# ToniChopp/ECAMP

Hardware: AMD Instinct MI355X
Metric: pretrain image-report pairs/sec (ViT-B/16, 224^2, seq=128) (higher is better)
Workload: dtype bf16

## Files before the change

ecamp_amd/csrc/attention.h:

```cpp
#pragma once
#include "common.h"

struct AttnArgs {
    const void* q; const void* k; const void* v; void* o;
    const void* dout; void* dq; void* dk; void* dv;
    float* lse; float* delta;
    const int32_t* key_mask;
    long q_sb, q_st, q_sh, k_sb, k_st, k_sh, v_sb, v_st, v_sh, o_sb, o_st, o_sh;
    long dq_sb, dq_st, dq_sh, dk_sb, dk_st, dk_sh, dv_sb, dv_st, dv_sh, do_sb, do_st, do_sh;
    int B, H, Tq, Tk;
    float scale, drop_p;
    uint64_t seed, offset;
    unsigned char* drop_bits;
};

#define NEG_BIG (-1.0e30f)

#define LDS_MAX (160 * 1024)

static inline int attn_kch(int Tk) { return Tk <= 64 ? 1 : Tk <= 128 ? 2 : Tk <= 256 ? 4 : 0; }

static inline size_t head_lds_bytes(int Tq, int Tk, int hd, bool backward, bool bits) {
    const int nkp = ((Tk + 15) / 16 + 1) / 2, nqp = ((Tq + 15) / 16 + 1) / 2;
    const size_t prow = (size_t)(backward && nqp > nkp ? nqp : nkp) * 32;
    return 2 * prow * (2 * hd) + (backward ? 3 : 1) * prow * sizeof(float) + (backward && bits ? 32 * prow : 0);
}

enum AttnFamily { ATTN_HEAD, ATTN_RESIDENT_FWD, ATTN_STREAM, ATTN_LONG, ATTN_F32 };
typedef void (*AttnKernel)(AttnArgs);
struct AttnLaunch {
    AttnFamily family;
    int n, block;
    struct Kernel { AttnKernel fn; dim3 grid; size_t lds, optin; } k[2];
};
#define ATTN_HD_SWITCH(hd, F, ...) ((hd) == 32 ? F<32>(__VA_ARGS__) : (hd) == 64 ? F<64>(__VA_ARGS__) : F<128>(__VA_ARGS__))

ECAMP_HIDDEN AttnLaunch attn16_select(int B, int H, int Tq, int Tk, int hd, bool mask_or_dropout, bool bits, bool backward);
ECAMP_HIDDEN void attn_launch(const AttnLaunch& l, const AttnArgs& a, hipStream_t st);
void attn_set_head_mode(int on);
```

ecamp_amd/csrc/attention.hip:

```cpp
#include "attention.h"


template <typename T, int HD, int PITCH>
__device__ __forceinline__ void stage_rows(float* dst, const T* base, long st, int r0, int nrows, int tid) {
    constexpr int V4 = HD / 4;
#pragma unroll
    for (int i = 0; i < (64 * V4) / 256; ++i) {
        int idx = tid + 256 * i;
        int row = idx / V4, dv = idx % V4;
        float p[4] = {0.f, 0.f, 0.f, 0.f};
        if (r0 + row < nrows) ld4<T>(base + (long)(r0 + row) * st + dv * 4, p);
        float* d = dst + row * PITCH + dv * 4;
        if (PITCH % 4 == 0) {
            *reinterpret_cast<float4*>(d) = make_float4(p[0], p[1], p[2], p[3]);
        } else {
            *reinterpret_cast<float2*>(d) = make_float2(p[0], p[1]);
            *reinterpret_cast<float2*>(d + 2) = make_float2(p[2], p[3]);
        }
    }
}

template <typename T, int HD>
__device__ __forceinline__ void load_rows_frag(float (&f)[HD / 4], const T* base, long st, int r0, int nrows, int lrow, int lk,
                                               float mul) {
// ... 450 lines not shown
                const int d = lane + 64 * t;
                if (d < HD) {
                    ak[t] = fmaf(di, qb[(long)(i0 + ii) * a.q_st + d], ak[t]);
                    av[t] = fmaf(pi, dOb[(long)(i0 + ii) * a.do_st + d], av[t]);
                }
            }
        }
    }
#pragma unroll
    for (int t = 0; t < (HD + 63) / 64; ++t) {
        const int d = lane + 64 * t;
        if (d < HD) { dk[d] = ak[t] * a.scale; dv[d] = av[t]; }
    }
}

static int attn_check(const AttnArgs& a, int hd, int dtype, bool bwd) {
    ECAMP_CHECK_ARG(hd == 32 || hd == 64 || hd == 128, "attention: head_dim %d not in {32,64,128}", hd);
    ECAMP_CHECK_ARG(a.Tk >= 1 && a.Tq >= 1, "attention: empty sequence");
    ECAMP_CHECK_ARG(dtype == ECAMP_F32 || dtype == ECAMP_BF16, "attention: bad dtype");
    ECAMP_CHECK_ARG(a.drop_p >= 0.f && a.drop_p < 1.f, "attention: bad dropout p");
    const long m = dtype == ECAMP_BF16 ? 8 : 4;
    if (dtype == ECAMP_BF16) ECAMP_CHECK_ARG(a.q_st % m == 0 && a.q_sb % m == 0 && a.q_sh % m == 0 && a.o_st % 4 == 0 && a.o_sb % 4 == 0 && a.o_sh % 4 == 0,
                                             "attention(bf16): q strides must be multiples of 8, o strides of 4 elements");
    ECAMP_CHECK_ARG(a.k_st % m == 0 && a.k_sb % m == 0 && a.k_sh % m == 0 && a.v_st % m == 0 && a.v_sb % m == 0 && a.v_sh % m == 0,
                    "attention: k/v strides must be multiples of 4 (f32) / 8 (bf16) elements");
    if (bwd) ECAMP_CHECK_ARG(a.q_st % m == 0 && a.q_sb % m == 0 && a.q_sh % m == 0 && a.do_st % m == 0 && a.do_sb % m == 0 && a.do_sh % m == 0,
                             "attention: q/dO strides must be multiples of 4 elements");
    return 0;
}

template <int HD>
static AttnLaunch select_f32(int B, int H, int Tq, int Tk, bool backward) {
    AttnLaunch l = {};
    l.family = ATTN_F32;
    l.n = backward ? 2 : 1;
    l.block = 256;
    const int kch = attn_kch(Tk);
    if (kch == 0) {
        const dim3 qrows((unsigned)(((long)B * H * Tq + 3) / 4)), krows((unsigned)(((long)B * H * Tk + 3) / 4));
        l.k[0] = {backward ? attn_long_bwd_dq_kernel<HD> : attn_long_fwd_kernel<HD>, qrows, 0, 0};
        if (backward) l.k[1] = {attn_long_bwd_dkv_kernel<HD>, krows, 0, 0};
        return l;
    }
    const dim3 qgrid(ceil_div(Tq, 64), B * H), kgrid(ceil_div(Tk, 64), B * H);
    const size_t fwd = (size_t)(64 * (HD + 16) + 4 * 16 * PP) * sizeof(float), dq = (size_t)(2 * 64 * (HD + 2) + 4 * 16 * PP) * sizeof(float),
                 dkv = (size_t)(2 * 64 * (HD + 2) + 8 * 16 * PP) * sizeof(float);
#define KCH_KERNEL(K) (kch == 1 ? K<float, HD, 1> : kch == 2 ? K<float, HD, 2> : K<float, HD, 4>)
    if (backward) {
        l.k[0] = {KCH_KERNEL(attn_bwd_dq_kernel), qgrid, dq, dq};
        l.k[1] = {attn_bwd_dkv_kernel<float, HD>, kgrid, dkv, dkv};
    } else {
        l.k[0] = {KCH_KERNEL(attn_fwd_kernel), qgrid, fwd, fwd};
    }
#undef KCH_KERNEL
    return l;
}
static AttnLaunch attn_select(int B, int H, int Tq, int Tk, int hd, int dtype, bool mask_or_dropout, bool bits, bool backward) {
    if (dtype == ECAMP_F32) return ATTN_HD_SWITCH(hd, select_f32, B, H, Tq, Tk, backward);
    return attn16_select(B, H, Tq, Tk, hd, mask_or_dropout, bits, backward);
}

static void stride3(long& sb, long& st, long& sh, const int64_t* s) {
    if (s) { sb = s[0]; st = s[1]; sh = s[2]; }
}
static AttnArgs attn_args(const void* q, const void* k, const void* v, const void* o, const void* dout, const float* lse, float* delta, void* dq,
                          void* dk, void* dv, const int32_t* key_mask, int32_t B, int32_t H, int32_t Tq, int32_t Tk, const int64_t* q_strides,
                          const int64_t* k_strides, const int64_t* v_strides, const int64_t* o_strides, const int64_t* do_strides,
                          const int64_t* dq_strides, const int64_t* dk_strides, const int64_t* dv_strides, float scale, float drop_p, uint64_t seed,
                          uint64_t offset, const void* drop_bits) {
    AttnArgs a;
    memset(&a, 0, sizeof(a));
    a.q = q; a.k = k; a.v = v; a.o = const_cast<void*>(o); a.dout = dout; a.lse = const_cast<float*>(lse); a.delta = delta;
    a.dq = dq; a.dk = dk; a.dv = dv; a.key_mask = key_mask;
    stride3(a.q_sb, a.q_st, a.q_sh, q_strides);
    stride3(a.k_sb, a.k_st, a.k_sh, k_strides);
    stride3(a.v_sb, a.v_st, a.v_sh, v_strides);
    stride3(a.o_sb, a.o_st, a.o_sh, o_strides);
    stride3(a.do_sb, a.do_st, a.do_sh, do_strides);
    stride3(a.dq_sb, a.dq_st, a.dq_sh, dq_strides);
    stride3(a.dk_sb, a.dk_st, a.dk_sh, dk_strides);
    stride3(a.dv_sb, a.dv_st, a.dv_sh, dv_strides);
    a.B = B; a.H = H; a.Tq = Tq; a.Tk = Tk; a.scale = scale; a.drop_p = drop_p; a.seed = seed; a.offset = offset;
    a.drop_bits = reinterpret_cast<unsigned char*>(const_cast<void*>(drop_bits));
    return a;
}

extern "C" int64_t ecamp_attn_mask_bytes(int32_t B, int32_t H, int32_t Tq, int32_t Tk, int32_t hd, int32_t dtype) {
    if (dtype != ECAMP_BF16 || B <= 0 || H <= 0 || Tq <= 0 || Tk <= 0 || Tk > 256) return 0;
    if (hd != 32 && hd != 64 && hd != 128) return 0;
    return ecamp_opt(OPT_ATTN_HEAD) != 0 && head_lds_bytes(Tq, Tk, hd, false, false) <= LDS_MAX ? (int64_t)B * H * Tq * 32 : 0;
}
extern "C" int ecamp_attn_fwd(const void* q, const void* k, const void* v, void* o, float* lse, const int32_t* key_mask,
                              int32_t B, int32_t H, int32_t Tq, int32_t Tk, int32_t hd, const int64_t* q_strides,
                              const int64_t* k_strides, const int64_t* v_strides, const int64_t* o_strides, float scale,
                              float drop_p, uint64_t seed, uint64_t offset, int32_t dtype, void* drop_mask, hipStream_t stream) {
    ECAMP_CHECK_ARG(q && k && v && o && lse && q_strides && k_strides && v_strides && o_strides, "attn_fwd: null pointer");
    const bool bits = dtype == ECAMP_BF16 && drop_p > 0.f && ecamp_attn_mask_bytes(B, H, Tq, Tk, hd, dtype) > 0;
    const AttnArgs a = attn_args(q, k, v, o, nullptr, lse, nullptr, nullptr, nullptr, nullptr, key_mask, B, H, Tq, Tk, q_strides, k_strides, v_strides,
                                 o_strides, nullptr, nullptr, nullptr, nullptr, scale, drop_p, seed, offset, bits ? drop_mask : nullptr);
    if (int rc = attn_check(a, hd, dtype, false)) return rc;
    const bool prof = ecamp_prof_active();
    if (prof) ecamp_prof_begin(ECAMP_PROF_ATTN, 4.0 * B * H * (double)Tq * Tk * hd, stream);
    attn_launch(attn_select(B, H, Tq, Tk, hd, dtype, key_mask != nullptr || drop_p > 0.f, a.drop_bits != nullptr, false), a, stream);
    if (prof) ecamp_prof_end(stream);
    ECAMP_LAUNCH_CHECK();
    return 0;
}

extern "C" int64_t ecamp_attn_bwd_workspace_bytes(int32_t B, int32_t H, int32_t Tq) { return (int64_t)B * H * Tq * 4; }

extern "C" int ecamp_attn_bwd(const void* q, const void* k, const void* v, const void* o, const void* dout, const float* lse,
                              float* delta_ws, void* dq, void* dk, void* dv, const int32_t* key_mask, int32_t B, int32_t H,
                              int32_t Tq, int32_t Tk, int32_t hd, const int64_t* q_strides, const int64_t* k_strides,
                              const int64_t* v_strides, const int64_t* o_strides, const int64_t* do_strides,
                              const int64_t* dq_strides, const int64_t* dk_strides, const int64_t* dv_strides, float scale,
                              float drop_p, uint64_t seed, uint64_t offset, int32_t dtype, const void* drop_mask, hipStream_t stream) {
    ECAMP_CHECK_ARG(q && k && v && o && dout && lse && delta_ws && dq && dk && dv && q_strides && k_strides && v_strides && o_strides && do_strides &&
                        dq_strides && dk_strides && dv_strides, "attn_bwd: null pointer");
    const bool bits = dtype == ECAMP_BF16 && drop_p > 0.f;
    const AttnArgs a = attn_args(q, k, v, o, dout, lse, delta_ws, dq, dk, dv, key_mask, B, H, Tq, Tk, q_strides, k_strides, v_strides, o_strides,
                                 do_strides, dq_strides, dk_strides, dv_strides, scale, drop_p, seed, offset, bits ? drop_mask : nullptr);
    if (int rc = attn_check(a, hd, dtype, true)) return rc;
    const bool prof = ecamp_prof_active();
    if (prof) ecamp_prof_begin(ECAMP_PROF_ATTN, 8.0 * B * H * (double)Tq * Tk * hd, stream);
    attn_launch(attn_select(B, H, Tq, Tk, hd, dtype, key_mask != nullptr || drop_p > 0.f, a.drop_bits != nullptr, true), a, stream);
    if (prof) ecamp_prof_end(stream);
    ECAMP_LAUNCH_CHECK();
    return 0;
}

template <typename T>
__global__ __launch_bounds__(256) void attn_probs_kernel(const T* __restrict__ q, const T* __restrict__ k, const int32_t* __restrict__ key_mask,
                                                         float* __restrict__ probs, int B, int H, int Tq, int Tk, int hd, long q_sb, long q_st,
                                                         long q_sh, long k_sb, long k_st, long k_sh, float scale) {
    const int lane = threadIdx.x & 63;
    const long row = (long)blockIdx.x * 4 + (threadIdx.x >> 6);
    if (row >= (long)B * H * Tq) return;
    const int i = (int)(row % Tq), h = (int)((row / Tq) % H), b = (int)(row / ((long)Tq * H));
    const T* qp = q + b * q_sb + i * q_st + h * q_sh;
    const T* kb = k + b * k_sb + h * k_sh;
    constexpr int MAXJ = 16;
    float s[MAXJ];
    float mx = -INFINITY;
#pragma unroll
    for (int jj = 0; jj < MAXJ; ++jj) {
        const int j = lane + 64 * jj;
        s[jj] = -INFINITY;
        if (j < Tk) {
            const T* kp = kb + (long)j * k_st;
            float acc = 0.f;
            for (int d = 0; d < hd; ++d) acc += to_f<T>(qp[d]) * to_f<T>(kp[d]);
            acc *= scale;
            if (key_mask && key_mask[(long)b * Tk + j] == 0) acc += -3.4028234663852886e38f;
            s[jj] = acc;
            mx = fmaxf(mx, acc);
        }
    }
    mx = wave_max(mx);
    float sum = 0.f;
#pragma unroll
    for (int jj = 0; jj < MAXJ; ++jj) {
        const int j = lane + 64 * jj;
        if (j < Tk) {
            s[jj] = __expf(s[jj] - mx);
            sum += s[jj];
        }
// ... 29 lines not shown
```

ecamp_amd/csrc/attention_bf16.hip:

```cpp
#include "attention.h"
#include <type_traits>

#ifdef ATTN_TS
__device__ long long attn_ts_buf[8 * 8192];
#define ATTN_STAMP(i) do { if (threadIdx.x == 0 && blockIdx.x < 8192) attn_ts_buf[blockIdx.x * 8 + (i)] = wall_clock64(); } while (0)
#else
#define ATTN_STAMP(i) do { } while (0)
#endif

typedef __attribute__((ext_vector_type(4))) short v4s16;
typedef hw_h16x8 bf16x8_t;

#define MFMA(a, b, c) ECAMP_MFMA_16x16x32(a, b, c)

#define ATTN_LOG2E 1.4426950408889634f
#define ATTN_LN2 0.6931471805599453f
__device__ __forceinline__ float attn_exp2(float x) { return __builtin_amdgcn_exp2f(x); }

template <int HD> struct TileCfg { static constexpr int PB = HD * 2 + 32; static constexpr int BYTES = 64 * PB; };

template <int HD>
__device__ __forceinline__ void stage_tile(unsigned char* lds, const bf16_t* base, long st, int r0, int nrows, int tid) {
    constexpr int CPR = HD / 8, PB = TileCfg<HD>::PB;
#pragma unroll
// ... 490 lines not shown
                    for (int r = 0; r < 4; ++r) p[r] *= dm[r];
                }
                ptile_write4(pt, li, jt * 16 + 4 * g, p);
            }
            __builtin_amdgcn_s_waitcnt(0xc07f);
            __builtin_amdgcn_wave_barrier();
#pragma unroll
            for (int kk = 0; kk < 2; ++kk) {
                bf16x8 pf = ptile_frag(pt, li, kk * 4 + g);
#pragma unroll
                for (int dt = 0; dt < HD / 16; ++dt) o[dt] = MFMA(frag_tr<HD>(VT + c * TB, dt * 16, kk * 32, lane), pf, o[dt]);
            }
            __builtin_amdgcn_s_waitcnt(0xc07f);
            __builtin_amdgcn_wave_barrier();
        }
        if (qi < a.Tq) {
#pragma unroll
            for (int dt = 0; dt < HD / 16; ++dt) store4(ob + (long)qi * a.o_st + dt * 16 + 4 * g, o[dt], 1.0f);
        }
    }
}

template <int HD> struct HeadCfg {
    static constexpr int RB = HD * 2, CPR = HD / 8;
    static constexpr unsigned long long KEYS = HD == 32 ? 0x3033030132330101ull : HD == 64 ? 0x6056142366024421ull : 0xE0CA8436CE0A3864ull;
};
template <int HD> __device__ __forceinline__ int hswz(int row) { return (int)((HeadCfg<HD>::KEYS >> (4 * (row & 15))) & 15ull); }
template <int HD> __device__ __forceinline__ unsigned haddr(int row, int chunk) {
    return (unsigned)(row * HeadCfg<HD>::RB + ((chunk ^ hswz<HD>(row)) << 4));
}
template <int HD>
__device__ __forceinline__ void head_stage(unsigned char* img, const bf16_t* base, long st, int nrows, int prow, int tid, int nthr) {
    constexpr int CPR = HeadCfg<HD>::CPR;
    const int n = prow * CPR;
    for (int i0 = tid; i0 < n; i0 += 4 * nthr) {
        uint4 v[4];
#pragma unroll
        for (int u = 0; u < 4; ++u) {
            const int idx = i0 + u * nthr, row = idx / CPR, ch = idx % CPR;
            v[u] = (idx < n && row < nrows) ? *reinterpret_cast<const uint4*>(base + (long)row * st + ch * 8) : make_uint4(0, 0, 0, 0);
        }
#pragma unroll
        for (int u = 0; u < 4; ++u) {
            const int idx = i0 + u * nthr, row = idx / CPR, ch = idx % CPR;
            if (idx < n) *reinterpret_cast<uint4*>(img + haddr<HD>(row, ch)) = v[u];
        }
    }
}
template <int HD, int U>
__device__ __forceinline__ void head_stage_pair(unsigned char* imgA, const bf16_t* baseA, long stA, unsigned char* imgB, const bf16_t* baseB, long stB,
                                                int nrows, int prow, int tid, int nthr) {
    constexpr int CPR = HeadCfg<HD>::CPR;
    const int n = prow * CPR;
    for (int i0 = tid; i0 < n; i0 += U * nthr) {
        uint4 va[U], vb[U];
#pragma unroll
        for (int u = 0; u < U; ++u) {
            const int idx = i0 + u * nthr, row = idx / CPR, ch = idx % CPR;
            const bool in = idx < n && row < nrows;
            va[u] = in ? *reinterpret_cast<const uint4*>(baseA + (long)row * stA + ch * 8) : make_uint4(0, 0, 0, 0);
            vb[u] = in ? *reinterpret_cast<const uint4*>(baseB + (long)row * stB + ch * 8) : make_uint4(0, 0, 0, 0);
        }
#pragma unroll
        for (int u = 0; u < U; ++u) {
            const int idx = i0 + u * nthr, row = idx / CPR, ch = idx % CPR;
            if (idx < n) {
                *reinterpret_cast<uint4*>(imgA + haddr<HD>(row, ch)) = va[u];
                *reinterpret_cast<uint4*>(imgB + haddr<HD>(row, ch)) = vb[u];
            }
        }
    }
}
typedef float f32x2 __attribute__((ext_vector_type(2)));
__device__ __forceinline__ f32x2 hexp2(f32x2 x) { return (f32x2){attn_exp2(x[0]), attn_exp2(x[1])}; }
__device__ __forceinline__ uint32_t hpk(f32x2 v) { return pack_bf16x2(v[0], v[1]); }
__device__ __forceinline__ bf16x8 hpack8(const float (&v)[8]) {
    const uint4 u = make_uint4(pack_bf16x2(v[0], v[1]), pack_bf16x2(v[2], v[3]), pack_bf16x2(v[4], v[5]), pack_bf16x2(v[6], v[7]));
    return __builtin_bit_cast(bf16x8, u);
}
__device__ __forceinline__ void head_key_bias(float* KB, const AttnArgs& a, int b, int prow, int tid, int nthr) {
    for (int j = tid; j < prow; j += nthr)
        KB[j] = (j < a.Tk && (a.key_mask == nullptr || a.key_mask[(long)b * a.Tk + j] != 0)) ? 0.f : NEG_BIG;
}
template <int HD> struct HeadOff {
    unsigned fr[HD / 32];
    unsigned tr[HD / 16];
    __device__ __forceinline__ HeadOff(int li, int g) {
#pragma unroll
        for (int ks = 0; ks < HD / 32; ++ks) fr[ks] = haddr<HD>(li, ks * 4 + g);
#pragma unroll
        for (int dt = 0; dt < HD / 16; ++dt) {
            const int cb = (dt * 16 + (li & 3) * 4) * 2;
            tr[dt] = haddr<HD>(4 * g + (li >> 2), cb >> 4) + (cb & 15);
        }
    }
};
template <int HD> __device__ __forceinline__ bf16x8 hfr(const unsigned char* img, const HeadOff<HD>& o, int t, int ks) {
    return *reinterpret_cast<const bf16x8*>(img + o.fr[ks] + t * (16 * HeadCfg<HD>::RB));
}
template <int HD> __device__ __forceinline__ bf16x8 htr(const unsigned char* img, const HeadOff<HD>& o, int pp, int dt) {
    const unsigned char* p = img + o.tr[dt] + pp * (32 * HeadCfg<HD>::RB);
    v4s16 lo = __builtin_amdgcn_ds_read_tr16_b64_v4i16((v4s16 __attribute__((address_space(3)))*)(p));
    v4s16 hi = __builtin_amdgcn_ds_read_tr16_b64_v4i16((v4s16 __attribute__((address_space(3)))*)(p + 16 * HeadCfg<HD>::RB));
    return (bf16x8){lo[0], lo[1], lo[2], lo[3], hi[0], hi[1], hi[2], hi[3]};
}

template <int HD, int FLAGS>
__global__ __launch_bounds__(512, 4) void attn_head_fwd_kernel(AttnArgs a) {
    extern __shared__ __attribute__((aligned(16))) unsigned char smem[];
    constexpr int RB = HeadCfg<HD>::RB;
    const int nthr = blockDim.x, nw = nthr >> 6;
    const int nkp = (((a.Tk + 15) >> 4) + 1) >> 1, prow = nkp * 32;
    const int pfull = FLAGS ? 0 : a.Tk >> 5;
    unsigned char* KI = smem;
    unsigned char* VI = smem + prow * RB;
    float* KB = reinterpret_cast<float*>(smem + 2 * prow * RB);
    const int tid = threadIdx.x, lane = tid & 63, wave = tid >> 6, li = lane & 15, g = lane >> 4;
    const int b = blockIdx.x / a.H, h = blockIdx.x % a.H;
    const long bh = blockIdx.x;
    const bf16_t* qb = reinterpret_cast<const bf16_t*>(a.q) + b * a.q_sb + h * a.q_sh;
    const bf16_t* kb = reinterpret_cast<const bf16_t*>(a.k) + b * a.k_sb + h * a.k_sh;
    const bf16_t* vb = reinterpret_cast<const bf16_t*>(a.v) + b * a.v_sb + h * a.v_sh;
    bf16_t* ob = reinterpret_cast<bf16_t*>(a.o) + b * a.o_sb + h * a.o_sh;
    bf16x8 qf[HD / 32];
    if (wave * 16 < a.Tq) load_row_frags<HD>(qf, qb, a.q_st, wave * 16, a.Tq, lane);
    head_stage_pair<HD, 4>(KI, kb, a.k_st, VI, vb, a.v_st, a.Tk, prow, tid, nthr);
    head_key_bias(KB, a, b, prow, tid, nthr);
    __syncthreads();
    const HeadOff<HD> off(li, g);
    const float sc2 = a.scale * ATTN_LOG2E;
    const float inv_keep = a.drop_p > 0.f ? 1.0f / (1.0f - a.drop_p) : 1.0f;
    for (int q0 = wave * 16; q0 < a.Tq; q0 += nw * 16) {
        auto scores = [&](int t, bool biased) {
            f32x4 acc = {0.f, 0.f, 0.f, 0.f};
#pragma unroll
            for (int ks = 0; ks < HD / 32; ++ks) acc = MFMA(hfr<HD>(KI, off, t, ks), qf[ks], acc);
            if (biased) {
                const f32x4 kb4 = *reinterpret_cast<const f32x4*>(KB + t * 16 + 4 * g);
#pragma unroll
                for (int r = 0; r < 4; ++r) acc[r] = fmaf(acc[r], sc2, kb4[r]);
            } else {
#pragma unroll
                for (int r = 0; r < 4; ++r) acc[r] *= sc2;
            }
            return acc;
        };
        float mx = NEG_BIG;
#pragma unroll 2
        for (int pp = 0; pp < pfull; ++pp) {
            const f32x4 s0 = scores(2 * pp, false), s1 = scores(2 * pp + 1, false);
            mx = fmaxf(fmaxf(fmaxf(mx, fmaxf(s0[0], s0[1])), fmaxf(s0[2], s0[3])), fmaxf(fmaxf(s1[0], s1[1]), fmaxf(s1[2], s1[3])));
        }
#pragma unroll 1
        for (int pp = pfull; pp < nkp; ++pp) {
            const f32x4 s0 = scores(2 * pp, true), s1 = scores(2 * pp + 1, true);
            mx = fmaxf(fmaxf(fmaxf(mx, fmaxf(s0[0], s0[1])), fmaxf(s0[2], s0[3])), fmaxf(fmaxf(s1[0], s1[1]), fmaxf(s1[2], s1[3])));
        }
        mx = red4_max(mx);
        const float mxs = fmaxf(mx, -1e29f);
        const int qi = q0 + li;
        float sum = 0.f;
        f32x4 o[HD / 16];
#pragma unroll
        for (int dt = 0; dt < HD / 16; ++dt) o[dt] = (f32x4){0.f, 0.f, 0.f, 0.f};
        auto pair = [&](int pp, bool biased) {
            const f32x4 s0 = scores(2 * pp, biased), s1 = scores(2 * pp + 1, biased);
            float p[8];
#pragma unroll
            for (int r = 0; r < 4; ++r) {
                p[r] = attn_exp2(s0[r] - mxs);
                p[4 + r] = attn_exp2(s1[r] - mxs);
                sum += p[r] + p[4 + r];
            }
            if (FLAGS && a.drop_p > 0.f) {
                float dm[4], dn[4];
                if ((a.Tk & 7) == 0) {
                    const bool odd = (g & 1) != 0;
                    const uint64_t e8 = ((((uint64_t)bh * a.Tq + qi) * (uint64_t)a.Tk) >> 3) + (uint64_t)(pp * 4 + (odd ? 2 : 0) + (g >> 1));
                    const uint4 P = philox4x32(a.seed, a.offset, e8);
                    const uint32_t r0 = (uint32_t)__builtin_amdgcn_ds_swizzle((int)(odd ? P.x : P.z), 0x401f);
                    const uint32_t r1 = (uint32_t)__builtin_amdgcn_ds_swizzle((int)(odd ? P.y : P.w), 0x401f);
                    const uint32_t wa0 = odd ? r0 : P.x, wa1 = odd ? r1 : P.y, wb0 = odd ? P.z : r0, wb1 = odd ? P.w : r1;
                    const uint32_t thr = dropout_thr(a.drop_p);
                    dm[0] = dropout_pick(wa0, 0, thr, inv_keep); dm[1] = dropout_pick(wa0, 1, thr, inv_keep);
                    dm[2] = dropout_pick(wa1, 0, thr, inv_keep); dm[3] = dropout_pick(wa1, 1, thr, inv_keep);
                    dn[0] = dropout_pick(wb0, 0, thr, inv_keep); dn[1] = dropout_pick(wb0, 1, thr, inv_keep);
                    dn[2] = dropout_pick(wb1, 0, thr, inv_keep); dn[3] = dropout_pick(wb1, 1, thr, inv_keep);
                } else {
                    attn_drop4(a, (uint64_t)bh * a.Tq + qi, pp * 32 + 4 * g, inv_keep, dm);
                    attn_drop4(a, (uint64_t)bh * a.Tq + qi, pp * 32 + 16 + 4 * g, inv_keep, dn);
                }
                unsigned bits = 0;
#pragma unroll
                for (int r = 0; r < 4; ++r) {
                    p[r] *= dm[r];
                    p[4 + r] *= dn[r];
                    bits |= (dm[r] != 0.f ? 1u << r : 0u) | (dn[r] != 0.f ? 16u << r : 0u);
                }
                if (a.drop_bits && qi < a.Tq) a.drop_bits[(((long)bh * a.Tq + qi) * 4 + g) * 8 + pp] = (unsigned char)bits;
            }
            const bf16x8 pf = hpack8(p);
#pragma unroll
            for (int dt = 0; dt < HD / 16; ++dt) o[dt] = MFMA(htr<HD>(VI, off, pp, dt), pf, o[dt]);
        };
#pragma unroll 2
        for (int pp = 0; pp < pfull; ++pp) pair(pp, false);
#pragma unroll 1
        for (int pp = pfull; pp < nkp; ++pp) pair(pp, true);
        sum = red4_sum(sum);
        if (qi < a.Tq) {
            if (g == 0) a.lse[bh * a.Tq + qi] = (mxs + __log2f(sum)) * ATTN_LN2;
            const float inv = sum > 0.f ? 1.0f / sum : 0.f;
#pragma unroll
            for (int dt = 0; dt < HD / 16; ++dt) store4(ob + (long)qi * a.o_st + dt * 16 + 4 * g, o[dt], inv);
        }
        if (q0 + nw * 16 < a.Tq) load_row_frags<HD>(qf, qb, a.q_st, q0 + nw * 16, a.Tq, lane);
    }
}

template <int HD, int FLAGS>
__global__ __launch_bounds__(256, (FLAGS == 0 && HD == 32) ? 5 : (FLAGS == 0 && HD == 64) ? 4 : 2) void attn_head_bwd_kernel(AttnArgs a) {
    extern __shared__ __attribute__((aligned(16))) unsigned char smem[];
    constexpr int RB = HeadCfg<HD>::RB;
    const int nthr = blockDim.x, nw = nthr >> 6;
    const int nkp = (((a.Tk + 15) >> 4) + 1) >> 1, nqp = (((a.Tq + 15) >> 4) + 1) >> 1, prow = max(nkp, nqp) * 32;
    const int pfull = FLAGS ? 0 : a.Tk >> 5;
    unsigned char* XI = smem;
    unsigned char* YI = smem + prow * RB;
    float* KB = reinterpret_cast<float*>(smem + 2 * prow * RB);
    float* LS = KB + prow;
    float* DL = LS + prow;
    unsigned char* MB = reinterpret_cast<unsigned char*>(DL + prow);
    const int tid = threadIdx.x, lane = tid & 63, wave = tid >> 6, li = lane & 15, g = lane >> 4;
    const int b = blockIdx.x / a.H, h = blockIdx.x % a.H;
    const long bh = blockIdx.x;
    const bool use_bits = FLAGS && a.drop_p > 0.f && a.drop_bits != nullptr;
    const bf16_t* qb = reinterpret_cast<const bf16_t*>(a.q) + b * a.q_sb + h * a.q_sh;
    const bf16_t* kb = reinterpret_cast<const bf16_t*>(a.k) + b * a.k_sb + h * a.k_sh;
    const bf16_t* vb = reinterpret_cast<const bf16_t*>(a.v) + b * a.v_sb + h * a.v_sh;
    const bf16_t* ob = reinterpret_cast<const bf16_t*>(a.o) + b * a.o_sb + h * a.o_sh;
    const bf16_t* gb = reinterpret_cast<const bf16_t*>(a.dout) + b * a.do_sb + h * a.do_sh;
    bf16_t* dqb = reinterpret_cast<bf16_t*>(a.dq) + b * a.dq_sb + h * a.dq_sh;
    bf16_t* dkb = reinterpret_cast<bf16_t*>(a.dk) + b * a.dk_sb + h * a.dk_sh;
    bf16_t* dvb = reinterpret_cast<bf16_t*>(a.dv) + b * a.dv_sb + h * a.dv_sh;
    const float sc2 = a.scale * ATTN_LOG2E;
    const float inv_keep = a.drop_p > 0.f ? 1.0f / (1.0f - a.drop_p) : 1.0f;
    const HeadOff<HD> off(li, g);

    ATTN_STAMP(0);
    bf16x8 qf[HD / 32], gf[HD / 32], of[HD / 32];
    float lse_c = 0.f;
    uint2 mw = make_uint2(0u, 0u);
    auto load_q = [&](int q0, bf16x8 (&q_)[HD / 32], bf16x8 (&g_)[HD / 32], bf16x8 (&o_)[HD / 32], float& l_) {
        load_row_frags<HD>(q_, qb, a.q_st, q0, a.Tq, lane);
        load_row_frags<HD>(g_, gb, a.do_st, q0, a.Tq, lane);
        load_row_frags<HD>(o_, ob, a.o_st, q0, a.Tq, lane);
        l_ = q0 + li < a.Tq ? a.lse[bh * a.Tq + q0 + li] : 0.f;
        if (use_bits && q0 + li < a.Tq) mw = *reinterpret_cast<const uint2*>(a.drop_bits + (((long)bh * a.Tq + q0 + li) * 4 + g) * 8);
    };
    if (wave * 16 < a.Tq) load_q(wave * 16, qf, gf, of, lse_c);
    head_stage_pair<HD, (HD == 128 ? 8 : 4)>(XI, kb, a.k_st, YI, vb, a.v_st, a.Tk, prow, tid, nthr);
    head_key_bias(KB, a, b, prow, tid, nthr);
    for (int i = ((a.Tq + 15) & ~15) + tid; i < prow; i += nthr) { LS[i] = 1e30f; DL[i] = 0.f; }
    __syncthreads();
    ATTN_STAMP(1);
    for (int q0 = wave * 16; q0 < a.Tq; q0 += nw * 16) {
        float dl = 0.f;
#pragma unroll
        for (int ks = 0; ks < HD / 32; ++ks)
#pragma unroll
            for (int e = 0; e < 8; ++e) dl += bf2f((bf16_t)gf[ks][e]) * bf2f((bf16_t)of[ks][e]);
        dl = red4_sum(dl);
        const int qi = q0 + li;
        const bool qok = qi < a.Tq;
        const float lse2 = qok ? lse_c * ATTN_LOG2E : 1e30f;
        if (g == 0) {
            LS[qi] = lse2;
            DL[qi] = qok ? dl : 0.f;
            if (qok && a.delta) a.delta[bh * a.Tq + qi] = dl;
        }
        f32x4 dq[HD / 16];
#pragma unroll
        for (int dt = 0; dt < HD / 16; ++dt) dq[dt] = (f32x4){0.f, 0.f, 0.f, 0.f};
        auto soft = [&](int pp, int hf, bool biased, const f32x4& s, const f32x4& dp, uint32_t& w0, uint32_t& w1) __attribute__((always_inline)) {
            const int t = 2 * pp + hf;
            f32x2 e0 = {s[0], s[1]}, e1 = {s[2], s[3]}, d0 = {dp[0], dp[1]}, d1 = {dp[2], dp[3]};
            const f32x2 sc = {sc2, sc2}, nl = {-lse2, -lse2}, dlv = {dl, dl};
            if (biased) {
                const f32x4 kb4 = *reinterpret_cast<const f32x4*>(KB + t * 16 + 4 * g);
                e0 = e0 * sc + ((f32x2){kb4[0], kb4[1]} + nl);
                e1 = e1 * sc + ((f32x2){kb4[2], kb4[3]} + nl);
            } else {
                e0 = e0 * sc + nl;
                e1 = e1 * sc + nl;
            }
            if (FLAGS && a.drop_p > 0.f) {
                float dm[4];
                if (use_bits) {
                    const unsigned nib = ((pp < 4 ? mw.x : mw.y) >> (8 * (pp & 3) + 4 * hf)) & 15u;
#pragma unroll
                    for (int r = 0; r < 4; ++r) dm[r] = (nib >> r) & 1u ? inv_keep : 0.f;
                } else {
                    attn_drop4(a, (uint64_t)bh * a.Tq + qi, t * 16 + 4 * g, inv_keep, dm);
                }
                d0 *= (f32x2){dm[0], dm[1]};
                d1 *= (f32x2){dm[2], dm[3]};
            }
            w0 = hpk(hexp2(e0) * (d0 - dlv));
            w1 = hpk(hexp2(e1) * (d1 - dlv));
        };
        auto pair = [&](int pp, bool biased) {
            uint32_t dsp[4];
            {
#pragma unroll
                for (int hf = 0; hf < 2; ++hf) {
                    const int t = 2 * pp + hf;
                    f32x4 s = {0.f, 0.f, 0.f, 0.f}, dp = {0.f, 0.f, 0.f, 0.f};
#pragma unroll
                    for (int ks = 0; ks < HD / 32; ++ks) {
                        s = MFMA(hfr<HD>(XI, off, t, ks), qf[ks], s);
                        dp = MFMA(hfr<HD>(YI, off, t, ks), gf[ks], dp);
                    }
                    soft(pp, hf, biased, s, dp, dsp[2 * hf], dsp[2 * hf + 1]);
                }
                const bf16x8 sf = __builtin_bit_cast(bf16x8, make_uint4(dsp[0], dsp[1], dsp[2], dsp[3]));
#pragma unroll
                for (int dt = 0; dt < HD / 16; ++dt) dq[dt] = MFMA(htr<HD>(XI, off, pp, dt), sf, dq[dt]);
            }
        };
#pragma unroll 2
        for (int pp = 0; pp < pfull; ++pp) pair(pp, false);
#pragma unroll 1
        for (int pp = pfull; pp < nkp; ++pp) pair(pp, true);
        if (qok) {
#pragma unroll
            for (int dt = 0; dt < HD / 16; ++dt) store4(dqb + (long)qi * a.dq_st + dt * 16 + 4 * g, dq[dt], a.scale);
        }
        if (q0 + nw * 16 < a.Tq) load_q(q0 + nw * 16, qf, gf, of, lse_c);
    }
    ATTN_STAMP(2);
    bf16x8 kf[HD / 32], vf[HD / 32];
    if (wave * 16 < a.Tk) {
        load_row_frags<HD>(kf, kb, a.k_st, wave * 16, a.Tk, lane);
        load_row_frags<HD>(vf, vb, a.v_st, wave * 16, a.Tk, lane);
    }
    __syncthreads();
    ATTN_STAMP(3);
    head_stage_pair<HD, (HD == 128 ? 8 : 4)>(XI, qb, a.q_st, YI, gb, a.do_st, a.Tq, prow, tid, nthr);
    if (use_bits) {
        for (int i = tid; i < a.Tq * 4; i += nthr) {
            const int row = i >> 2, gg = i & 3;
            const uint2 w = *reinterpret_cast<const uint2*>(a.drop_bits + ((long)bh * a.Tq * 4 + i) * 8);
#pragma unroll
            for (int pp = 0; pp < 8; ++pp) MB[(gg * 8 + pp) * prow + row] = (unsigned char)(((pp < 4 ? w.x : w.y) >> (8 * (pp & 3))) & 255u);
        }
    }
    __syncthreads();
    ATTN_STAMP(4);
    for (int j0 = wave * 16; j0 < a.Tk; j0 += nw * 16) {
        const int kj = j0 + li;
        const bool jok = KB[kj] == 0.f;
        const f32x2 kb2 = {KB[kj], KB[kj]};
        const unsigned char* mcol = MB + ((((kj & 15) >> 2) * 8 + (kj >> 5)) * prow);
        const int mbit = 4 * ((kj >> 4) & 1) + (kj & 3);
        f32x4 dk[HD / 16], dv[HD / 16];
#pragma unroll
        for (int dt = 0; dt < HD / 16; ++dt) dk[dt] = dv[dt] = (f32x4){0.f, 0.f, 0.f, 0.f};
#pragma unroll 2
        for (int ip = 0; ip < nqp; ++ip) {
            uint32_t pdp[4], dsp[4];
            auto soft2 = [&](int hf, const f32x4& s, const f32x4& dp) __attribute__((always_inline)) {
                const int it = 2 * ip + hf;
                const f32x4 lse4 = *reinterpret_cast<const f32x4*>(LS + it * 16 + 4 * g);
                const f32x4 dl4 = *reinterpret_cast<const f32x4*>(DL + it * 16 + 4 * g);
                const f32x2 sc = {sc2, sc2};
                f32x2 d0 = {dp[0], dp[1]}, d1 = {dp[2], dp[3]};
                f32x2 e0 = (f32x2){s[0], s[1]} * sc - (f32x2){lse4[0], lse4[1]}, e1 = (f32x2){s[2], s[3]} * sc - (f32x2){lse4[2], lse4[3]};
                if (FLAGS) { e0 += kb2; e1 += kb2; }
                f32x2 p0 = hexp2(e0);
                f32x2 p1 = hexp2(e1);
                if (FLAGS && a.drop_p > 0.f) {
                    float dm[4];
                    if (use_bits) {
                        const unsigned m4 = *reinterpret_cast<const unsigned*>(mcol + it * 16 + 4 * g) >> mbit;
#pragma unroll
                        for (int r = 0; r < 4; ++r) dm[r] = (m4 >> (8 * r)) & 1u ? inv_keep : 0.f;
                    } else {
                        attn_drop4_col(a, (uint64_t)bh * a.Tq + (it * 16 + 4 * g), kj, li, inv_keep, dm);
                    }
                    const f32x2 m0 = {dm[0], dm[1]}, m1 = {dm[2], dm[3]};
                    d0 *= m0; d1 *= m1;
                    pdp[2 * hf] = hpk(p0 * m0);
                    pdp[2 * hf + 1] = hpk(p1 * m1);
                } else {
                    pdp[2 * hf] = hpk(p0);
                    pdp[2 * hf + 1] = hpk(p1);
                }
                dsp[2 * hf] = hpk(p0 * (d0 - (f32x2){dl4[0], dl4[1]}));
                dsp[2 * hf + 1] = hpk(p1 * (d1 - (f32x2){dl4[2], dl4[3]}));
            };
            {
#pragma unroll
                for (int hf = 0; hf < 2; ++hf) {
                    const int it = 2 * ip + hf;
                    f32x4 s = {0.f, 0.f, 0.f, 0.f}, dp = {0.f, 0.f, 0.f, 0.f};
#pragma unroll
                    for (int ks = 0; ks < HD / 32; ++ks) {
                        s = MFMA(hfr<HD>(XI, off, it, ks), kf[ks], s);
                        dp = MFMA(hfr<HD>(YI, off, it, ks), vf[ks], dp);
                    }
                    soft2(hf, s, dp);
                }
                const bf16x8 pf = __builtin_bit_cast(bf16x8, make_uint4(pdp[0], pdp[1], pdp[2], pdp[3]));
                const bf16x8 sf = __builtin_bit_cast(bf16x8, make_uint4(dsp[0], dsp[1], dsp[2], dsp[3]));
#pragma unroll
                for (int dt = 0; dt < HD / 16; ++dt) {
                    dv[dt] = MFMA(htr<HD>(YI, off, ip, dt), pf, dv[dt]);
                    dk[dt] = MFMA(htr<HD>(XI, off, ip, dt), sf, dk[dt]);
                }
            }
        }
        if (kj < a.Tk) {
            const float mk = jok ? a.scale : 0.f, mv = jok ? 1.0f : 0.f;
#pragma unroll
            for (int dt = 0; dt < HD / 16; ++dt) {
                store4(dkb + (long)kj * a.dk_st + dt * 16 + 4 * g, dk[dt], mk);
                store4(dvb + (long)kj * a.dv_st + dt * 16 + 4 * g, dv[dt], mv);
            }
        }
        if (j0 + nw * 16 < a.Tk) {
            load_row_frags<HD>(kf, kb, a.k_st, j0 + nw * 16, a.Tk, lane);
            load_row_frags<HD>(vf, vb, a.v_st, j0 + nw * 16, a.Tk, lane);
        }
    }
    ATTN_STAMP(5);
}

static long g_head_launches = 0;
extern "C" int64_t ecamp_attn_head_launches(void) { return g_head_launches; }
void attn_set_head_mode(int on) { ecamp_opt_set("attn_head", on); }
static int head_waves(int tiles, int cap) {
    const int env = ecamp_opt(OPT_ATTN_WAVES);
    if (env > 0) cap = env;
    return tiles < cap ? tiles : cap;
}
template <int HD>
static AttnLaunch select16(int B, int H, int Tq, int Tk, bool flags, bool bits, bool backward) {
    static_assert(HeadCfg<HD>::RB == 2 * HD, "head_lds_bytes (attention.h) states the row size of the head images");
    AttnLaunch l = {};
    l.n = 1;
    l.block = 256;
    const int nqt = (Tq + 15) / 16, nkt = (Tk + 15) / 16;
    const size_t head = head_lds_bytes(Tq, Tk, HD, backward, bits);
    if (ecamp_opt(OPT_ATTN_HEAD) != 0 && head <= LDS_MAX) {
        l.family = ATTN_HEAD;
        l.block = 64 * (backward ? head_waves(nkt > nqt ? nkt : nqt, 4) : head_waves(nqt, 8));
        const AttnKernel fn = backward ? (flags ? attn_head_bwd_kernel<HD, 1> : attn_head_bwd_kernel<HD, 0>)
                                       : (flags ? attn_head_fwd_kernel<HD, 1> : attn_head_fwd_kernel<HD, 0>);
        l.k[0] = {fn, dim3(B * H), head, LDS_MAX};
        return l;
    }
    const dim3 qgrid(ceil_div(Tq, 64), B * H), kgrid(ceil_div(Tk, 64), B * H);
    const size_t stream = (size_t)2 * TileCfg<HD>::BYTES + 4 * 2048 + 64 * sizeof(int);
    const int kch = attn_kch(Tk);
    if (backward) {
        l.family = ATTN_STREAM;
        l.n = 2;
        const AttnKernel dq = kch == 1 ? attn16_bwd_dq_kernel<HD, 1> : kch == 2 ? attn16_bwd_dq_kernel<HD, 2> : kch == 4 ? attn16_bwd_dq_kernel<HD, 4>
                                                                                                                       : attn16_bwd_dq_kernel<HD, 0>;
        l.k[0] = {dq, qgrid, stream, 0};
        l.k[1] = {attn16_bwd_dkv_kernel<HD>, kgrid, (size_t)2 * TileCfg<HD>::BYTES + 8 * 2048 + 128 * sizeof(float), 0};
        return l;
    }
    if (Tk > 128) {
        l.family = ATTN_LONG;
        l.k[0] = {attn16_fwd_long_kernel<HD>, qgrid, stream, 0};
        return l;
    }
    l.family = ATTN_RESIDENT_FWD;
    const size_t shm = (size_t)2 * kch * TileCfg<HD>::BYTES + 4 * 2048;
    l.k[0] = {kch == 1 ? attn16r_fwd_kernel<HD, 1> : attn16r_fwd_kernel<HD, 2>, dim3(B * H), shm, shm};
    return l;
}
AttnLaunch attn16_select(int B, int H, int Tq, int Tk, int hd, bool mask_or_dropout, bool bits, bool backward) {
    return ATTN_HD_SWITCH(hd, select16, B, H, Tq, Tk, mask_or_dropout, bits, backward);
}

void attn_launch(const AttnLaunch& l, const AttnArgs& a, hipStream_t st) {
    static const void* seen[64];
    static int n_seen = 0;
    for (int i = 0; i < l.n; ++i) {
        const AttnLaunch::Kernel& k = l.k[i];
        const void* fn = reinterpret_cast<const void*>(k.fn);
        bool known = k.optin <= 48 * 1024;
        for (int s = 0; s < n_seen && !known; ++s) known = seen[s] == fn;
        if (!known) {
            (void)hipFuncSetAttribute(fn, hipFuncAttributeMaxDynamicSharedMemorySize, (int)k.optin);
            if (n_seen < 64) seen[n_seen++] = fn;
        }
        hipLaunchKernelGGL(k.fn, k.grid, dim3(l.block), k.lds, st, a);
    }
    if (l.family == ATTN_HEAD) ++g_head_launches;
}
```

ecamp_amd/csrc/core.hip:

```cpp
#include "common.h"
#include "attention.h"
#include "options.h"
#include "../../include/ecamp_hip.h"
#include <atomic>
#include <stdarg.h>
#include <stdlib.h>

thread_local char g_ecamp_err[512] = {0};

int ecamp_set_error(int code, const char* fmt, ...) {
    va_list ap;
    va_start(ap, fmt);
    vsnprintf(g_ecamp_err, sizeof(g_ecamp_err), fmt, ap);
    va_end(ap);
    return code;
}

extern "C" const char* ecamp_last_error(void) { return g_ecamp_err; }
extern "C" int ecamp_abi_version(void) { return ECAMP_ABI_VERSION; }
extern "C" int ecamp_half_format(void) { return ECAMP_HALF_IS_F16; }

#define OPT_UNREAD (INT_MIN + 1)
struct OptRow {
    const char* name; const char* env; int def; int (*set)(int);
    std::atomic<int> value{OPT_ENV};
    std::atomic<int> env_value{OPT_UNREAD};
};
static OptRow g_opts[OPT_COUNT] = {
              {"q8_mode", "ECAMP_GEMM_Q8", -1, [](int v) { return v == 0 || v == 2 ? v : -1; }},
               {"q8_sch", "ECAMP_Q8_SCH", 7, [](int v) { return v >= 0 ? v : OPT_ENV; }},
             {"q16_mode", "ECAMP_Q16", 1, [](int v) { return v >= 0 && v <= 3 ? v : OPT_ENV; }},
                {nullptr, "ECAMP_F8_Q8", 1, nullptr},
         {nullptr, "ECAMP_Q8_MIN_ITEMS", OPT_AUTO, nullptr},
          {"q8_bwd_grid", "ECAMP_Q8_BWD_GRID", 0, [](int v) { return v > 0 ? v : OPT_ENV; }},
             {"p8_wgrad", nullptr, 1, [](int v) { return v ? 1 : 0; }},
     {"p8_wgrad_reserve_cus", nullptr, 0, [](int v) { return v < 0 ? 0 : v; }},
          {nullptr, "ECAMP_WGRAD_ITEMS", 0, nullptr},
           {nullptr, "ECAMP_WGRAD_PLAN", 1, nullptr},
      {nullptr, "ECAMP_WGRAD_GROUP_CUS", 0, nullptr},
        {nullptr, "ECAMP_GEMM_GRID_CAP", 0, nullptr},
            {"attn_head", "ECAMP_ATTN_HEAD", 1, [](int v) { return v < 0 ? OPT_ENV : v ? 1 : 0; }},
           {nullptr, "ECAMP_ATTN_WAVES", 0, nullptr},
               {nullptr, "ECAMP_LN_BWD", 0, nullptr},
            {nullptr, "ECAMP_CE_KERNEL", 1, nullptr},
            {nullptr, "ECAMP_SR_BLOCKS", 512, nullptr},
};
int ecamp_opt_default(EcampOpt id) { return g_opts[id].def; }
int ecamp_opt(EcampOpt id) {
    OptRow& o = g_opts[id];
    const int s = o.value.load(std::memory_order_relaxed);
    if (s != OPT_ENV) return s;
    int e = o.env_value.load(std::memory_order_relaxed);
    if (e == OPT_UNREAD) {
        const char* txt = o.env ? getenv(o.env) : nullptr;
        e = txt ? atoi(txt) : o.def;
        o.env_value.store(e, std::memory_order_relaxed);
    }
    return e;
}
bool ecamp_opt_set(const char* name, int value) {
    for (OptRow& o : g_opts)
        if (o.name && strcmp(name, o.name) == 0) {
            o.value.store(o.set(value), std::memory_order_relaxed);
            return true;
        }
    return false;
}
extern "C" int ecamp_set_option(const char* name, int32_t value) {
    ECAMP_CHECK_ARG(name != nullptr, "set_option: null name");
    if (strcmp(name, "attn_head") == 0) { attn_set_head_mode(value); return 0; }
    if (ecamp_opt_set(name, value)) return 0;
    return ecamp_set_error(-1, "set_option: unknown option '%s'", name);
}

__global__ void dev_spin_kernel(long long cycles) {
    const long long t0 = clock64();
    while (clock64() - t0 < cycles) {}
}
extern "C" int ecamp_dev_spin(int32_t blocks, int32_t threads, int64_t cycles, hipStream_t stream) {
    ECAMP_CHECK_ARG(blocks > 0 && threads > 0 && threads <= 1024 && cycles >= 0, "dev_spin: bad arguments");
    hipLaunchKernelGGL(dev_spin_kernel, dim3(blocks), dim3(threads), 0, stream, (long long)cycles);
    ECAMP_LAUNCH_CHECK();
    return 0;
}
```

ecamp_amd/csrc/options.h:

```cpp
#pragma once
#include <limits.h>

enum EcampOpt {
    OPT_Q8_MODE, OPT_Q8_SCH, OPT_Q16_MODE, OPT_F8_Q8, OPT_Q8_MIN_ITEMS, OPT_Q8_BWD_GRID, OPT_P8_WGRAD, OPT_P8_WGRAD_RESERVE,
    OPT_WGRAD_ITEMS, OPT_WGRAD_PLAN, OPT_WGRAD_GROUP_CUS, OPT_GEMM_GRID_CAP, OPT_ATTN_HEAD, OPT_ATTN_WAVES, OPT_LN_BWD, OPT_CE_KERNEL,
    OPT_SR_BLOCKS, OPT_COUNT
};
#define OPT_ENV INT_MIN
#define OPT_AUTO INT_MIN

#define ECAMP_HIDDEN __attribute__((visibility("hidden")))
ECAMP_HIDDEN int ecamp_opt(EcampOpt id);
ECAMP_HIDDEN int ecamp_opt_default(EcampOpt id);
ECAMP_HIDDEN bool ecamp_opt_set(const char* name, int value);
```

Baseline: 7380.

## Skip trailing padded key blocks in per-head attention forward and backward

Adds an option, on by default, under which the per-head attention kernels compute the last unmasked key position from the key-padding mask. They then stage, score and backpropagate only the key tiles up to that point. Gradients for the padded keys are written as zeros directly, and rows whose logsumexp is -inf are guarded. This targets wasted work on padded text tokens (seq=128 reports are often shorter), at the cost of an extra sync and ballot scan before staging. Dropout bit generation still covers all tiles when bits are saved.

```diff
diff --git a/ecamp_amd/csrc/attention.h b/ecamp_amd/csrc/attention.h
--- a/ecamp_amd/csrc/attention.h
+++ b/ecamp_amd/csrc/attention.h
@@ -12,6 +12,7 @@
     float scale, drop_p;
     uint64_t seed, offset;
     unsigned char* drop_bits;
+    int skip_masked;
 };
 
 #define NEG_BIG (-1.0e30f)
diff --git a/ecamp_amd/csrc/attention.hip b/ecamp_amd/csrc/attention.hip
--- a/ecamp_amd/csrc/attention.hip
+++ b/ecamp_amd/csrc/attention.hip
@@ -556,6 +556,7 @@
     stride3(a.dv_sb, a.dv_st, a.dv_sh, dv_strides);
     a.B = B; a.H = H; a.Tq = Tq; a.Tk = Tk; a.scale = scale; a.drop_p = drop_p; a.seed = seed; a.offset = offset;
     a.drop_bits = reinterpret_cast<unsigned char*>(const_cast<void*>(drop_bits));
+    a.skip_masked = ecamp_opt(OPT_ATTN_SKIP_MASKED) != 0;
     return a;
 }
 
diff --git a/ecamp_amd/csrc/attention_bf16.hip b/ecamp_amd/csrc/attention_bf16.hip
--- a/ecamp_amd/csrc/attention_bf16.hip
+++ b/ecamp_amd/csrc/attention_bf16.hip
@@ -596,6 +596,14 @@
     for (int j = tid; j < prow; j += nthr)
         KB[j] = (j < a.Tk && (a.key_mask == nullptr || a.key_mask[(long)b * a.Tk + j] != 0)) ? 0.f : NEG_BIG;
 }
+__device__ __forceinline__ int head_key_end(const float* KB, int prow, int lane) {
+    int end = 0;
+    for (int j0 = 0; j0 < prow; j0 += 64) {
+        const unsigned long long m = __ballot(j0 + lane < prow && KB[j0 + lane] == 0.f);
+        if (m) end = j0 + 64 - __builtin_clzll(m);
+    }
+    return __builtin_amdgcn_readfirstlane(end);
+}
 template <int HD> struct HeadOff {
     unsigned fr[HD / 32];
     unsigned tr[HD / 16];
@@ -638,8 +646,15 @@
     bf16_t* ob = reinterpret_cast<bf16_t*>(a.o) + b * a.o_sb + h * a.o_sh;
     bf16x8 qf[HD / 32];
     if (wave * 16 < a.Tq) load_row_frags<HD>(qf, qb, a.q_st, wave * 16, a.Tq, lane);
-    head_stage_pair<HD, 4>(KI, kb, a.k_st, VI, vb, a.v_st, a.Tk, prow, tid, nthr);
-    head_key_bias(KB, a, b, prow, tid, nthr);
+    const bool skip = FLAGS && a.skip_masked;
+    int npl = nkp;
+    if (skip) {
+        head_key_bias(KB, a, b, prow, tid, nthr);
+        __syncthreads();
+        npl = (head_key_end(KB, prow, lane) + 31) >> 5;
+    }
+    head_stage_pair<HD, 4>(KI, kb, a.k_st, VI, vb, a.v_st, a.Tk, npl * 32, tid, nthr);
+    if (!skip) head_key_bias(KB, a, b, prow, tid, nthr);
     __syncthreads();
     const HeadOff<HD> off(li, g);
     const float sc2 = a.scale * ATTN_LOG2E;
@@ -666,7 +681,7 @@
             mx = fmaxf(fmaxf(fmaxf(mx, fmaxf(s0[0], s0[1])), fmaxf(s0[2], s0[3])), fmaxf(fmaxf(s1[0], s1[1]), fmaxf(s1[2], s1[3])));
         }
 #pragma unroll 1
-        for (int pp = pfull; pp < nkp; ++pp) {
+        for (int pp = pfull; pp < npl; ++pp) {
             const f32x4 s0 = scores(2 * pp, true), s1 = scores(2 * pp + 1, true);
             mx = fmaxf(fmaxf(fmaxf(mx, fmaxf(s0[0], s0[1])), fmaxf(s0[2], s0[3])), fmaxf(fmaxf(s1[0], s1[1]), fmaxf(s1[2], s1[3])));
         }
@@ -677,50 +692,60 @@
         f32x4 o[HD / 16];
 #pragma unroll
         for (int dt = 0; dt < HD / 16; ++dt) o[dt] = (f32x4){0.f, 0.f, 0.f, 0.f};
+        auto keep8 = [&](int pp, float (&dm)[4], float (&dn)[4]) __attribute__((always_inline)) {
+            if ((a.Tk & 7) == 0) {
+                const bool odd = (g & 1) != 0;
+                const uint64_t e8 = ((((uint64_t)bh * a.Tq + qi) * (uint64_t)a.Tk) >> 3) + (uint64_t)(pp * 4 + (odd ? 2 : 0) + (g >> 1));
+                const uint4 P = philox4x32(a.seed, a.offset, e8);
+                const uint32_t r0 = (uint32_t)__builtin_amdgcn_ds_swizzle((int)(odd ? P.x : P.z), 0x401f);
+                const uint32_t r1 = (uint32_t)__builtin_amdgcn_ds_swizzle((int)(odd ? P.y : P.w), 0x401f);
+                const uint32_t wa0 = odd ? r0 : P.x, wa1 = odd ? r1 : P.y, wb0 = odd ? P.z : r0, wb1 = odd ? P.w : r1;
+                const uint32_t thr = dropout_thr(a.drop_p);
+                dm[0] = dropout_pick(wa0, 0, thr, inv_keep); dm[1] = dropout_pick(wa0, 1, thr, inv_keep);
+                dm[2] = dropout_pick(wa1, 0, thr, inv_keep); dm[3] = dropout_pick(wa1, 1, thr, inv_keep);
+                dn[0] = dropout_pick(wb0, 0, thr, inv_keep); dn[1] = dropout_pick(wb0, 1, thr, inv_keep);
+                dn[2] = dropout_pick(wb1, 0, thr, inv_keep); dn[3] = dropout_pick(wb1, 1, thr, inv_keep);
+            } else {
+                attn_drop4(a, (uint64_t)bh * a.Tq + qi, pp * 32 + 4 * g, inv_keep, dm);
+                attn_drop4(a, (uint64_t)bh * a.Tq + qi, pp * 32 + 16 + 4 * g, inv_keep, dn);
+            }
+            unsigned bits = 0;
+#pragma unroll
+            for (int r = 0; r < 4; ++r) bits |= (dm[r] != 0.f ? 1u << r : 0u) | (dn[r] != 0.f ? 16u << r : 0u);
+            if (a.drop_bits && qi < a.Tq) a.drop_bits[(((long)bh * a.Tq + qi) * 4 + g) * 8 + pp] = (unsigned char)bits;
+        };
         auto pair = [&](int pp, bool biased) {
-            const f32x4 s0 = scores(2 * pp, biased), s1 = scores(2 * pp + 1, biased);
-            float p[8];
-#pragma unroll
-            for (int r = 0; r < 4; ++r) {
-                p[r] = attn_exp2(s0[r] - mxs);
-                p[4 + r] = attn_exp2(s1[r] - mxs);
-                sum += p[r] + p[4 + r];
+            const bool live = !FLAGS || pp < npl;
+            float p[8] = {0.f, 0.f, 0.f, 0.f, 0.f, 0.f, 0.f, 0.f};
+            if (live) {
+                const f32x4 s0 = scores(2 * pp, biased), s1 = scores(2 * pp + 1, biased);
+#pragma unroll
+                for (int r = 0; r < 4; ++r) {
+                    p[r] = attn_exp2(s0[r] - mxs);
+                    p[4 + r] = attn_exp2(s1[r] - mxs);
+                    sum += p[r] + p[4 + r];
+                }
             }
             if (FLAGS && a.drop_p > 0.f) {
                 float dm[4], dn[4];
-                if ((a.Tk & 7) == 0) {
-                    const bool odd = (g & 1) != 0;
-                    const uint64_t e8 = ((((uint64_t)bh * a.Tq + qi) * (uint64_t)a.Tk) >> 3) + (uint64_t)(pp * 4 + (odd ? 2 : 0) + (g >> 1));
-                    const uint4 P = philox4x32(a.seed, a.offset, e8);
-                    const uint32_t r0 = (uint32_t)__builtin_amdgcn_ds_swizzle((int)(odd ? P.x : P.z), 0x401f);
-                    const uint32_t r1 = (uint32_t)__builtin_amdgcn_ds_swizzle((int)(odd ? P.y : P.w), 0x401f);
-                    const uint32_t wa0 = odd ? r0 : P.x, wa1 = odd ? r1 : P.y, wb0 = odd ? P.z : r0, wb1 = odd ? P.w : r1;
-                    const uint32_t thr = dropout_thr(a.drop_p);
-                    dm[0] = dropout_pick(wa0, 0, thr, inv_keep); dm[1] = dropout_pick(wa0, 1, thr, inv_keep);
-                    dm[2] = dropout_pick(wa1, 0, thr, inv_keep); dm[3] = dropout_pick(wa1, 1, thr, inv_keep);
-                    dn[0] = dropout_pick(wb0, 0, thr, inv_keep); dn[1] = dropout_pick(wb0, 1, thr, inv_keep);
-                    dn[2] = dropout_pick(wb1, 0, thr, inv_keep); dn[3] = dropout_pick(wb1, 1, thr, inv_keep);
-                } else {
-                    attn_drop4(a, (uint64_t)bh * a.Tq + qi, pp * 32 + 4 * g, inv_keep, dm);
-                    attn_drop4(a, (uint64_t)bh * a.Tq + qi, pp * 32 + 16 + 4 * g, inv_keep, dn);
-                }
-                unsigned bits = 0;
+                keep8(pp, dm, dn);
 #pragma unroll
                 for (int r = 0; r < 4; ++r) {
                     p[r] *= dm[r];
                     p[4 + r] *= dn[r];
-                    bits |= (dm[r] != 0.f ? 1u << r : 0u) | (dn[r] != 0.f ? 16u << r : 0u);
                 }
-                if (a.drop_bits && qi < a.Tq) a.drop_bits[(((long)bh * a.Tq + qi) * 4 + g) * 8 + pp] = (unsigned char)bits;
-            }
-            const bf16x8 pf = hpack8(p);
-#pragma unroll
-            for (int dt = 0; dt < HD / 16; ++dt) o[dt] = MFMA(htr<HD>(VI, off, pp, dt), pf, o[dt]);
+            }
+            if (live) {
+                const bf16x8 pf = hpack8(p);
+#pragma unroll
+                for (int dt = 0; dt < HD / 16; ++dt) o[dt] = MFMA(htr<HD>(VI, off, pp, dt), pf, o[dt]);
+            }
         };
 #pragma unroll 2
         for (int pp = 0; pp < pfull; ++pp) pair(pp, false);
+        const int npb = FLAGS && a.drop_p > 0.f && a.drop_bits ? nkp : npl;
 #pragma unroll 1
-        for (int pp = pfull; pp < nkp; ++pp) pair(pp, true);
+        for (int pp = pfull; pp < npb; ++pp) pair(pp, true);
         sum = red4_sum(sum);
         if (qi < a.Tq) {
             if (g == 0) a.lse[bh * a.Tq + qi] = (mxs + __log2f(sum)) * ATTN_LN2;
@@ -773,8 +798,17 @@
         if (use_bits && q0 + li < a.Tq) mw = *reinterpret_cast<const uint2*>(a.drop_bits + (((long)bh * a.Tq + q0 + li) * 4 + g) * 8);
     };
     if (wave * 16 < a.Tq) load_q(wave * 16, qf, gf, of, lse_c);
-    head_stage_pair<HD, (HD == 128 ? 8 : 4)>(XI, kb, a.k_st, YI, vb, a.v_st, a.Tk, prow, tid, nthr);
-    head_key_bias(KB, a, b, prow, tid, nthr);
+    const bool skip = FLAGS && a.skip_masked;
+    int klive = a.Tk, npl = nkp, krow = prow;
+    if (skip) {
+        head_key_bias(KB, a, b, prow, tid, nthr);
+        __syncthreads();
+        klive = head_key_end(KB, prow, lane);
+        npl = (klive + 31) >> 5;
+        krow = npl * 32;
+    }
+    head_stage_pair<HD, (HD == 128 ? 8 : 4)>(XI, kb, a.k_st, YI, vb, a.v_st, a.Tk, krow, tid, nthr);
+    if (!skip) head_key_bias(KB, a, b, prow, tid, nthr);
     for (int i = ((a.Tq + 15) & ~15) + tid; i < prow; i += nthr) { LS[i] = 1e30f; DL[i] = 0.f; }
     __syncthreads();
     ATTN_STAMP(1);
@@ -787,7 +821,7 @@
         dl = red4_sum(dl);
         const int qi = q0 + li;
         const bool qok = qi < a.Tq;
-        const float lse2 = qok ? lse_c * ATTN_LOG2E : 1e30f;
+        const float lse2 = qok && !(FLAGS && lse_c == -INFINITY) ? lse_c * ATTN_LOG2E : 1e30f;
         if (g == 0) {
             LS[qi] = lse2;
             DL[qi] = qok ? dl : 0.f;
@@ -845,7 +879,7 @@
 #pragma unroll 2
         for (int pp = 0; pp < pfull; ++pp) pair(pp, false);
 #pragma unroll 1
-        for (int pp = pfull; pp < nkp; ++pp) pair(pp, true);
+        for (int pp = pfull; pp < npl; ++pp) pair(pp, true);
         if (qok) {
 #pragma unroll
             for (int dt = 0; dt < HD / 16; ++dt) store4(dqb + (long)qi * a.dq_st + dt * 16 + 4 * g, dq[dt], a.scale);
@@ -854,7 +888,7 @@
     }
     ATTN_STAMP(2);
     bf16x8 kf[HD / 32], vf[HD / 32];
-    if (wave * 16 < a.Tk) {
+    if (wave * 16 < klive) {
         load_row_frags<HD>(kf, kb, a.k_st, wave * 16, a.Tk, lane);
         load_row_frags<HD>(vf, vb, a.v_st, wave * 16, a.Tk, lane);
     }
@@ -866,12 +900,21 @@
             const int row = i >> 2, gg = i & 3;
             const uint2 w = *reinterpret_cast<const uint2*>(a.drop_bits + ((long)bh * a.Tq * 4 + i) * 8);
 #pragma unroll
-            for (int pp = 0; pp < 8; ++pp) MB[(gg * 8 + pp) * prow + row] = (unsigned char)(((pp < 4 ? w.x : w.y) >> (8 * (pp & 3))) & 255u);
+            for (int pp = 0; pp < 8; ++pp)
+                if (pp < npl) MB[(gg * 8 + pp) * prow + row] = (unsigned char)(((pp < 4 ? w.x : w.y) >> (8 * (pp & 3))) & 255u);
         }
     }
     __syncthreads();
     ATTN_STAMP(4);
-    for (int j0 = wave * 16; j0 < a.Tk; j0 += nw * 16) {
+    if (FLAGS) {
+        const int z0 = (klive + 15) & ~15;
+        for (int i = tid; i < (a.Tk - z0) * (HD / 4); i += nthr) {
+            const long kj = z0 + i / (HD / 4), c = (i % (HD / 4)) * 4;
+            *reinterpret_cast<uint2*>(dkb + kj * a.dk_st + c) = make_uint2(0u, 0u);
+            *reinterpret_cast<uint2*>(dvb + kj * a.dv_st + c) = make_uint2(0u, 0u);
+        }
+    }
+    for (int j0 = wave * 16; j0 < klive; j0 += nw * 16) {
         const int kj = j0 + li;
         const bool jok = KB[kj] == 0.f;
         const f32x2 kb2 = {KB[kj], KB[kj]};
@@ -942,7 +985,7 @@
                 store4(dvb + (long)kj * a.dv_st + dt * 16 + 4 * g, dv[dt], mv);
             }
         }
-        if (j0 + nw * 16 < a.Tk) {
+        if (j0 + nw * 16 < klive) {
             load_row_frags<HD>(kf, kb, a.k_st, j0 + nw * 16, a.Tk, lane);
             load_row_frags<HD>(vf, vb, a.v_st, j0 + nw * 16, a.Tk, lane);
         }
diff --git a/ecamp_amd/csrc/core.hip b/ecamp_amd/csrc/core.hip
--- a/ecamp_amd/csrc/core.hip
+++ b/ecamp_amd/csrc/core.hip
@@ -41,6 +41,7 @@
         {nullptr, "ECAMP_GEMM_GRID_CAP", 0, nullptr},
             {"attn_head", "ECAMP_ATTN_HEAD", 1, [](int v) { return v < 0 ? OPT_ENV : v ? 1 : 0; }},
            {nullptr, "ECAMP_ATTN_WAVES", 0, nullptr},
+     {"attn_skip_masked", "ECAMP_ATTN_SKIP_MASKED", 1, [](int v) { return v < 0 ? OPT_ENV : v ? 1 : 0; }},
                {nullptr, "ECAMP_LN_BWD", 0, nullptr},
             {nullptr, "ECAMP_CE_KERNEL", 1, nullptr},
             {nullptr, "ECAMP_SR_BLOCKS", 512, nullptr},
diff --git a/ecamp_amd/csrc/options.h b/ecamp_amd/csrc/options.h
--- a/ecamp_amd/csrc/options.h
+++ b/ecamp_amd/csrc/options.h
@@ -3,7 +3,7 @@
 
 enum EcampOpt {
     OPT_Q8_MODE, OPT_Q8_SCH, OPT_Q16_MODE, OPT_F8_Q8, OPT_Q8_MIN_ITEMS, OPT_Q8_BWD_GRID, OPT_P8_WGRAD, OPT_P8_WGRAD_RESERVE,
-    OPT_WGRAD_ITEMS, OPT_WGRAD_PLAN, OPT_WGRAD_GROUP_CUS, OPT_GEMM_GRID_CAP, OPT_ATTN_HEAD, OPT_ATTN_WAVES, OPT_LN_BWD, OPT_CE_KERNEL,
+    OPT_WGRAD_ITEMS, OPT_WGRAD_PLAN, OPT_WGRAD_GROUP_CUS, OPT_GEMM_GRID_CAP, OPT_ATTN_HEAD, OPT_ATTN_WAVES, OPT_ATTN_SKIP_MASKED, OPT_LN_BWD, OPT_CE_KERNEL,
     OPT_SR_BLOCKS, OPT_COUNT
 };
 #define OPT_ENV INT_MIN
```

Result: no change. 7404 (median of 6 runs) (+0.3%).
